# SJTU-ViSYS-team/Avoid-MPC

Hardware: AMD Instinct MI355X
Metric: MPC steps/sec (50k-pt cloud, N=20, 8 obstacle constraints) (higher is better)
Workload: dtype f64; 1 GPU; BASELINE configs[1] batched as configs[2]: 256 scenes/GPU x (50000-pt obstacle cloud + 5000-pt edge cloud, N=20, K=8), fresh frame + zero warm start every step, every in-flight step on its own frames; scenes_per_gpu=256, points=50000, horizon=20, K=8, mpc_max_iter=3, ipm_max_iter=100, streams_in_flight=10, steps_per_launch=4, scenes_per_launch=1024, distinct_frames_bytes=6758400000, hw_queues=4, tie_order=lowest index, parallelism=single GPU, no process group, rccl=no process group (single GPU, plain run): RCCL not used

## Files before the change

avoid_mpc_amd/capi.py:

```python
import ctypes as C
import os

HERE = os.path.dirname(os.path.abspath(__file__))
LIB_PATH = os.path.join(HERE, "libavoid_mpc_amd.so")

AMK_OK, AMK_ERR_INVALID_ARG, AMK_ERR_HIP, AMK_ERR_NO_DEVICE, AMK_ERR_UNSUPPORTED, AMK_ERR_TIMEOUT = 0, 1, 2, 3, 4, 5
AMK_TIES_LOWEST_INDEX, AMK_TIES_NANOFLANN, AMK_TIES_AUTO = 0, 1, 2
AMK_EXACT_OFF, AMK_EXACT_IN_USE, AMK_EXACT_GAVE_UP, AMK_EXACT_TOO_DEEP = -1, 0, 1, 2
AMK_EXACT_NOT_NEEDED = 3
AMK_MAX_K = 64
AMK_MAX_QUERIES = 64
AMK_MAX_HORIZON = 32
AMK_MAX_OUTER_ITER = 8
AMK_MPC_DEFAULT_MAX_ITER = 100

PLUGIN_FUNCTIONS = ["nlp", "nlp_f", "nlp_g", "nlp_grad_f", "nlp_jac_g", "nlp_hess_l", "nlp_grad"]
PLUGIN_HELPERS = ["alloc_mem", "init_mem", "free_mem", "checkout", "release", "incref", "decref", "n_in", "n_out",
                  "default_in", "name_in", "name_out", "sparsity_in", "sparsity_out", "work"]
PLUGIN_SYMBOLS = [f for f in PLUGIN_FUNCTIONS] + [f + "_" + h for f in PLUGIN_FUNCTIONS for h in PLUGIN_HELPERS] + \
                 ["amk_plugin_configure", "amk_plugin_dims"]

SYMBOLS = [
    "amk_version", "amk_status_string", "amk_last_hip_error", "amk_device_count",
    "amk_kd_create", "amk_kd_destroy", "amk_kd_build", "amk_kd_build_pair", "amk_kd_sizes", "amk_kd_search",
    "amk_kd_build_host", "amk_kd_search_host", "amk_kd_tie_flags", "amk_kd_set_tie_order", "amk_kd_exact_status", "amk_kd_exact_status_host", "amk_kd_keyframe_sweep",
    "amk_kd_keyframe_sweep_host", "amk_kd_points_host",
    "amk_mpc_create", "amk_mpc_destroy", "amk_mpc_horizon", "amk_mpc_nx", "amk_mpc_ref_len",
    "amk_mpc_setup_weights", "amk_mpc_setup_tau", "amk_mpc_setup_gains", "amk_mpc_set_drag_coefficient", "amk_mpc_set_drone_radius",
    "amk_kfmap_pool_bytes", "amk_kfmap_create", "amk_kfmap_destroy", "amk_kfmap_reset", "amk_kfmap_scenes", "amk_kfmap_frames", "amk_kfmap_twc", "amk_kfmap_add_vertex",
    "amk_kfmap_update", "amk_kfmap_step", "amk_kfmap_state_host",
    "amk_kfmap_set_tie_order", "amk_kfmap_tie_order_bytes", "amk_kfmap_exact_status_host",
    "amk_kfmap_query_nearest", "amk_kfmap_nearest_distance", "amk_kfmap_query_nearest_host", "amk_kfmap_nearest_distance_host",
    "amk_kfmap_points_host", "amk_kd_query_frames", "amk_kd_nearest_distance_frames", "amk_kd_query_frames_host",
    "amk_mpc_set_drone_accel_limits", "amk_mpc_set_solver_options", "amk_mpc_set_solve_budget", "amk_mpc_set_precision", "amk_mpc_solve",
    "amk_mpc_get_warm_start", "amk_mpc_set_warm_start", "amk_mpc_reset_warm_start",
    "amk_mpc_solve_host", "amk_mpc_ng", "amk_mpc_jac_nnz", "amk_mpc_hess_nnz", "amk_mpc_jac_sparsity",
    "amk_mpc_hess_sparsity", "amk_mpc_eval", "amk_mpc_eval_host", "amk_mpc_np", "amk_mpc_eval_gamma",
    "amk_mpc_eval_gamma_host", "amk_step_batch", "amk_step_batch_frames", "amk_step_batch_host",
    "amk_pipeline_create", "amk_pipeline_destroy", "amk_pipeline_slots", "amk_pipeline_gang", "amk_pipeline_mpc", "amk_pipeline_kd",
    "amk_pipeline_kfmap",
    "amk_pipeline_stream", "amk_pipeline_submit", "amk_pipeline_wait", "amk_pipeline_query", "amk_pipeline_drain",
    "amk_pipeline_outputs", "amk_pipeline_wait_stream",
    "amk_shard_scene_range", "amk_shard_unique_id", "amk_shard_create", "amk_shard_destroy", "amk_shard_rank",
    "amk_shard_world", "amk_shard_last_rccl_error", "amk_shard_gather", "amk_shard_gather_u", "amk_shard_max", "amk_shard_padded_count",
    "amk_shard_rccl_info", "amk_shard_wait",
    "amk_depth_out_size", "amk_depth_to_cloud", "amk_depth_to_cloud_host",
    "amk_depth_to_edge_cloud", "amk_depth_to_edge_cloud_host",
]


class AmkError(RuntimeError):
    pass


class StepParams(C.Structure):
    _fields_ = [("speed", C.c_double), ("safety_distance", C.c_double),
                ("mpc_max_iter", C.c_int), ("reserved", C.c_int)]


class DepthParams(C.Structure):
    _fields_ = [("pixel2meter", C.c_double), ("depth_min", C.c_double), ("depth_max", C.c_double),
                ("resize_scale", C.c_double), ("fx", C.c_double), ("fy", C.c_double), ("cx", C.c_double),
                ("cy", C.c_double), ("Tbc", C.c_double * 16)]


class TaskParams(C.Structure):
    _fields_ = [("decay", C.c_double), ("iter_time", C.c_double), ("farest_point", C.c_double), ("height", C.c_double),
                ("slow_down_kp", C.c_double), ("slow_down_kd", C.c_double), ("a_max_xy", C.c_double), ("a_max_z", C.c_double),
                ("use_odom_est", C.c_int), ("task", C.c_int)]


class KfmapParams(C.Structure):
    _fields_ = [("max_frame_count", C.c_int), ("keyframe_th_count", C.c_int), ("keyframe_th_dist", C.c_double), ("depth_min", C.c_double),
                ("Tbc", C.c_double * 16)]


class PipelineConfig(C.Structure):
    _fields_ = [("n_slots", C.c_int), ("n_scenes", C.c_int), ("max_points", C.c_int), ("max_edge_points", C.c_int),
                ("T", C.c_double), ("dt", C.c_double), ("nearest_point_num", C.c_int), ("queue_depth", C.c_int),
                ("gang", C.c_int), ("step", StepParams), ("task", TaskParams), ("depth", DepthParams), ("keyframes", KfmapParams)]


class PipelineFrame(C.Structure):
    _fields_ = [("d_cloud", C.c_void_p), ("d_cloud_counts", C.c_void_p), ("d_edge", C.c_void_p), ("d_edge_counts", C.c_void_p),
                ("point_stride", C.c_int), ("keep_warm_start", C.c_int), ("d_state_quad", C.c_void_p), ("d_pos_x", C.c_void_p),
                ("d_ref_path_init", C.c_void_p), ("d_u_out", C.c_void_p), ("d_odom", C.c_void_p), ("odom_age", C.c_double),
                ("d_cmd_out", C.c_void_p), ("d_depth", C.c_void_p), ("depth_type", C.c_int), ("depth_rows", C.c_int), ("depth_cols", C.c_int),
                ("reserved", C.c_int), ("d_Twb", C.c_void_p), ("kf_obstacle", C.c_void_p), ("kf_edge", C.c_void_p), ("n_keyframes", C.c_int),
                ("reserved2", C.c_int), ("d_Twc_cur", C.c_void_p), ("camera", C.c_void_p), ("input_ready", C.c_void_p),
                ("d_global_goal", C.c_void_p)]


class FrameCamera(C.Structure):
    _fields_ = [("fx", C.c_double), ("fy", C.c_double), ("cx", C.c_double), ("cy", C.c_double),
                ("depth_max", C.c_double), ("width", C.c_int), ("height", C.c_int)]


AMK_DEPTH_U16, AMK_DEPTH_F32 = 0, 1

_lib = None


def load():
    global _lib
    if _lib is not None:
        return _lib
    if not os.path.exists(LIB_PATH):
        raise AmkError(f"{LIB_PATH} is missing: build it with `python -m avoid_mpc_amd.build` "
                       "(hipcc, gfx950).  There is no CPU fallback.")
    try:
        import torch
    except ImportError:
        pass
    lib = C.CDLL(LIB_PATH)
    vp, i, d, ll = C.c_void_p, C.c_int, C.c_double, C.c_longlong
    sig = {
        "amk_version": (i, []),
        "amk_status_string": (C.c_char_p, [i]),
        "amk_last_hip_error": (i, []),
        "amk_device_count": (i, []),
        "amk_kd_create": (i, [i, i, C.POINTER(vp)]),
        "amk_kd_destroy": (i, [vp]),
        "amk_kd_build": (i, [vp, vp, i, ll, vp, vp]),
        "amk_kd_build_pair": (i, [vp, vp, vp, vp, vp, vp, i, vp]),
        "amk_kd_sizes": (i, [vp, vp, vp]),
        "amk_kd_search": (i, [vp, vp, i, i, vp, vp, vp, vp, vp]),
        "amk_kd_tie_flags": (i, [vp, vp, i, i, i, vp, vp]),
        "amk_kd_set_tie_order": (i, [vp, i]),
        "amk_kd_exact_status": (i, [vp, vp, vp]),
        "amk_kd_exact_status_host": (i, [vp, vp]),
        "amk_kd_keyframe_sweep": (i, [vp, vp, d, i, vp, vp, vp]),
        "amk_kd_keyframe_sweep_host": (i, [vp, vp, d, i, vp, vp]),
        "amk_kd_points_host": (i, [vp, vp, vp]),
        "amk_kd_build_host": (i, [vp, vp, i, ll, vp]),
        "amk_kd_search_host": (i, [vp, vp, i, i, vp, vp, vp, vp]),
        "amk_mpc_create": (i, [d, d, i, i, C.POINTER(vp)]),
        "amk_mpc_destroy": (i, [vp]),
        "amk_mpc_horizon": (i, [vp]),
        "amk_mpc_nx": (i, [vp]),
        "amk_mpc_ref_len": (i, [vp]),
        "amk_mpc_setup_weights": (i, [vp, vp]),
        "amk_mpc_setup_tau": (i, [vp, vp]),
        "amk_mpc_setup_gains": (i, [vp, vp]),
        "amk_mpc_set_drag_coefficient": (i, [vp, d, d, d]),
        "amk_mpc_set_drone_radius": (i, [vp, d]),
        "amk_mpc_set_drone_accel_limits": (i, [vp, d, d, d, d]),
        "amk_mpc_set_solver_options": (i, [vp, d, i]),
        "amk_mpc_set_precision": (i, [vp, i]),
        "amk_mpc_solve": (i, [vp, vp, vp, vp, vp, i, vp]),
        "amk_mpc_get_warm_start": (i, [vp, vp, vp]),
        "amk_mpc_set_warm_start": (i, [vp, vp, vp]),
        "amk_mpc_reset_warm_start": (i, [vp, vp]),
        "amk_mpc_solve_host": (i, [vp, vp, vp, vp, vp, i]),
        "amk_mpc_ng": (i, [vp]),
        "amk_mpc_jac_nnz": (i, [vp]),
        "amk_mpc_hess_nnz": (i, [vp]),
        "amk_mpc_jac_sparsity": (i, [vp, vp, vp]),
        "amk_mpc_hess_sparsity": (i, [vp, vp, vp]),
        "amk_mpc_eval": (i, [vp, vp, vp, vp, vp, vp, vp, vp, vp, vp]),
        "amk_mpc_eval_host": (i, [vp, vp, vp, vp, vp, vp, vp, vp, vp]),
        "amk_mpc_np": (i, [vp]),
        "amk_mpc_eval_gamma": (i, [vp, vp, vp, vp, vp, vp, vp, vp]),
        "amk_mpc_eval_gamma_host": (i, [vp, vp, vp, vp, vp, vp, vp]),
        "amk_step_batch": (i, [vp, vp, vp, C.POINTER(StepParams), vp, vp, vp, vp, vp, vp, vp]),
        "amk_step_batch_host": (i, [vp, vp, vp, C.POINTER(StepParams), vp, vp, vp, vp, vp, vp]),
        "amk_step_batch_frames": (i, [vp, vp, i, vp, C.POINTER(FrameCamera), vp, C.POINTER(StepParams), vp, vp, vp, vp, vp,
                                      vp, vp]),
        "amk_pipeline_create": (i, [C.POINTER(PipelineConfig), C.POINTER(vp)]),
        "amk_pipeline_destroy": (i, [vp]),
        "amk_pipeline_slots": (i, [vp]),
        "amk_mpc_set_solve_budget": (i, [vp, i, i]),
        "amk_pipeline_gang": (i, [vp]),
        "amk_pipeline_mpc": (vp, [vp, i]),
        "amk_pipeline_kd": (vp, [vp, i, i]),
        "amk_pipeline_kfmap": (vp, [vp, i]),
        "amk_pipeline_stream": (vp, [vp, i]),
        "amk_pipeline_submit": (i, [vp, C.POINTER(PipelineFrame), C.POINTER(i)]),
        "amk_pipeline_wait": (i, [vp, i]),
        "amk_pipeline_wait_stream": (i, [vp, i, vp]),
        "amk__pipeline_inject_failure": (i, [vp, i]),
        "amk_pipeline_query": (i, [vp, i]),
        "amk_pipeline_drain": (i, [vp]),
        "amk_pipeline_outputs": (i, [vp, i, C.POINTER(vp), C.POINTER(vp), C.POINTER(vp), C.POINTER(vp)]),
        "amk_kfmap_pool_bytes": (i, [i, i, i, i, C.POINTER(C.c_longlong)]),
        "amk_kfmap_create": (i, [i, i, i, C.POINTER(KfmapParams), C.POINTER(vp)]),
        "amk_kfmap_destroy": (i, [vp]),
        "amk_kfmap_reset": (i, [vp, i, i, vp]),
        "amk_kfmap_scenes": (i, [vp]),
        "amk_kfmap_frames": (i, [vp]),
        "amk_kfmap_twc": (vp, [vp]),
        "amk_kfmap_add_vertex": (i, [vp, i, i, vp, vp, vp, vp, i, vp, vp]),
        "amk_kfmap_update": (i, [vp, vp]),
        "amk_kfmap_step": (i, [vp, vp, vp, C.POINTER(StepParams), vp, vp, vp, vp, vp, vp, vp]),
        "amk_kfmap_state_host": (i, [vp, vp, vp, vp, vp]),
        "amk_kfmap_set_tie_order": (i, [vp, i]),
        "amk_kfmap_tie_order_bytes": (i, [i, i, i, i, C.POINTER(C.c_longlong)]),
        "amk_kfmap_exact_status_host": (i, [vp, vp, vp]),
        "amk_kfmap_query_nearest": (i, [vp, C.POINTER(FrameCamera), vp, i, i, i, i, vp, vp, vp, vp, vp]),
        "amk_kfmap_nearest_distance": (i, [vp, vp, i, i, vp, vp]),
        "amk_kfmap_query_nearest_host": (i, [vp, C.POINTER(FrameCamera), vp, i, i, i, i, vp, vp, vp, vp]),
        "amk_kfmap_nearest_distance_host": (i, [vp, vp, i, i, vp]),
        "amk_kfmap_points_host": (i, [vp, i, vp, ll, vp, C.POINTER(ll)]),
        "amk_kd_query_frames": (i, [vp, i, vp, C.POINTER(FrameCamera), vp, i, i, i, vp, vp, vp, vp, vp]),
        "amk_kd_nearest_distance_frames": (i, [vp, i, vp, i, i, vp, vp]),
        "amk_kd_query_frames_host": (i, [vp, i, vp, C.POINTER(FrameCamera), vp, i, i, i, vp, vp, vp, vp]),
        "amk_shard_scene_range": (i, [i, i, i, C.POINTER(i), C.POINTER(i)]),
        "amk_shard_unique_id": (i, [C.c_char_p]),
        "amk_shard_create": (i, [C.c_char_p, i, i, C.POINTER(vp)]),
        "amk_shard_destroy": (i, [vp]),
        "amk_shard_rank": (i, [vp]),
        "amk_shard_world": (i, [vp]),
        "amk_shard_last_rccl_error": (i, []),
        "amk_shard_gather": (i, [vp, vp, ll, vp, vp]),
        "amk_shard_gather_u": (i, [vp, vp, i, vp, vp]),
        "amk_shard_max": (i, [vp, vp, i, vp]),
        "amk_shard_padded_count": (i, [i, i]),
        "amk_shard_rccl_info": (i, [C.c_char_p, i, C.POINTER(i), C.POINTER(i)]),
        "amk_shard_wait": (i, [vp, vp, d]),
        "amk_depth_out_size": (i, [i, i, d, C.POINTER(i), C.POINTER(i)]),
        "amk_depth_to_cloud": (i, [vp, i, i, i, C.c_longlong, i, C.POINTER(DepthParams), vp, vp, i, C.c_longlong, vp, vp]),
        "amk_depth_to_cloud_host": (i, [vp, i, i, i, C.c_longlong, i, C.POINTER(DepthParams), vp, vp, i, C.c_longlong, vp]),
        "amk_depth_to_edge_cloud": (i, [vp, i, i, i, C.c_longlong, i, C.POINTER(DepthParams), vp, vp, i, C.c_longlong, vp, vp]),
        "amk_depth_to_edge_cloud_host": (i, [vp, i, i, i, C.c_longlong, i, C.POINTER(DepthParams), vp, vp, i, C.c_longlong, vp]),
    }
    sig["amk__kd_set_mode"] = (i, [vp, i])
    sig["amk__sweep_set_target"] = (None, [i])
    sig["amk__sweep_set_order"] = (None, [i])
    sig["amk__frames_force_wide"] = (None, [i])
    sig["amk__mpc_ref_states"] = (i, [vp, vp, ll])
    sig["amk__kfmap_slots_host"] = (i, [vp, vp, vp, vp, vp, vp])
    for name, (res, args) in sig.items():
        fn = getattr(lib, name, None)
        if fn is None:
# ... 60 lines not shown
```

avoid_mpc_amd/csrc/pipeline.hip:

```cpp
#include "mpc_handle.h"

#include <chrono>
#include <cstdlib>
#include <cstring>
#include <vector>

struct amk_pipeline {
    amk_pipeline_config cfg;
    struct Staged {
        amk_pipeline_frame frame;
        std::vector<amk_kd *> kf_obstacle, kf_edge;
        bool has_camera = false;
        amk_frame_camera camera{};
        hipEvent_t input_ready = nullptr;
    };
    struct Slot {
        hipStream_t stream = nullptr;
        std::vector<hipEvent_t> done;
        long long count = 0;
        long long waited = 0;
        amk_kd *obstacle = nullptr, *edge = nullptr;
        amk_mpc *mpc = nullptr;
        amk::DevBuf<double> ref_path, u, x0array, state_quad, pos_x;
        amk::DevBuf<int> flags;
        std::vector<Staged> open;
        int point_stride = 3;
        amk::DevBuf<float> dcloud, dedge;
        amk::DevBuf<int> dcount, decount;
        amk::DevBuf<double> Twc;
        bool ref_inited[AMK_PIPELINE_MAX_GANG] = {};
        amk_kfmap *map = nullptr;
        int fail_status = AMK_OK;
    };
    int depth = 1, gang = 1;
    std::vector<Slot> slots;
    int next = 0;
    long long submitted = 0;
    int inject_failure = 0;
};

namespace {
struct GatherArgs {
    const double *sq[AMK_PIPELINE_MAX_GANG], *px[AMK_PIPELINE_MAX_GANG], *ref[AMK_PIPELINE_MAX_GANG];
    int keep_warm_start[AMK_PIPELINE_MAX_GANG];
    double *sq_dst, *px_dst, *ref_dst, *w0;
    int n_sq, n_px, n_ref, n_w0;
};
__global__ __launch_bounds__(256) void pipeline_gather_kernel(const GatherArgs a) {
    const int g = blockIdx.y;
    const int stride = gridDim.x * 256, t0 = blockIdx.x * 256 + threadIdx.x;
    if (a.sq_dst && a.sq[g]) {
        for (int i = t0; i < a.n_sq; i += stride) a.sq_dst[(size_t)g * a.n_sq + i] = a.sq[g][i];
        for (int i = t0; i < a.n_px; i += stride) a.px_dst[(size_t)g * a.n_px + i] = a.px[g][i];
    }
    if (a.ref[g])
        for (int i = t0; i < a.n_ref; i += stride) a.ref_dst[(size_t)g * a.n_ref + i] = a.ref[g][i];
    if (!a.keep_warm_start[g])
        for (int i = t0; i < a.n_w0; i += stride) a.w0[(size_t)g * a.n_w0 + i] = 0.0;
}
struct ScatterArgs {
    double *dst[AMK_PIPELINE_MAX_GANG];
    double *cmd[AMK_PIPELINE_MAX_GANG];
    const double *odom[AMK_PIPELINE_MAX_GANG];
    const double *u;
    const int *flags;
    int n_u, S;
    double kp, kd, a_max_xy, a_max_z;
};
__global__ __launch_bounds__(256) void pipeline_scatter_kernel(const ScatterArgs a) {
#pragma clang fp contract(off)
    const int g = blockIdx.y;
    if (a.dst[g] && a.dst[g] != a.u + (size_t)g * a.n_u)
        for (int i = blockIdx.x * 256 + threadIdx.x; i < a.n_u; i += gridDim.x * 256) a.dst[g][i] = a.u[(size_t)g * a.n_u + i];
    if (a.cmd[g]) {
        for (int i = blockIdx.x * 256 + threadIdx.x; i < a.S * 3; i += gridDim.x * 256) {
            const int s = i / 3, c = i - 3 * s;
            const size_t gs = (size_t)g * a.S + s;
            double v;
            if (a.flags[gs * 4 + 0]) v = a.u[gs * 4 + c];
            else {
                const double *o = a.odom[g] + (size_t)s * 10;
                v = -o[4 + c] * a.kp - o[7 + c] * a.kd + (c == 2 ? 9.8 : 0.0);
                const double lim = c == 2 ? a.a_max_z : a.a_max_xy;
                v = fmax(-lim, fmin(lim, v));
            }
            a.cmd[g][i] = v;
        }
    }
}

__global__ __launch_bounds__(256) void pipeline_twc_update_kernel(const double *__restrict__ Twb, const int *__restrict__ counts,
                                                                  double *__restrict__ Twc, int S, const amk_depth_params prm) {
// ... 248 lines not shown
            sa.dst[g] = f.d_u_out; sa.cmd[g] = f.d_odom ? f.d_cmd_out : nullptr; sa.odom[g] = f.d_odom;
            any = any || sa.dst[g] || sa.cmd[g];
        }
        sa.u = s.u.p; sa.flags = s.flags.p; sa.n_u = S * 4; sa.S = S;
        sa.kp = c.task.slow_down_kp; sa.kd = c.task.slow_down_kd; sa.a_max_xy = c.task.a_max_xy; sa.a_max_z = c.task.a_max_z;
        if (any) {
            hipLaunchKernelGGL(pipeline_scatter_kernel, dim3((sa.n_u + 255) / 256 > 16 ? 16 : (sa.n_u + 255) / 256, filled), dim3(256), 0, st, sa);
            AMK_HIP(hipGetLastError());
        }
    }
    AMK_HIP(hipEventRecord(s.done[s.count % p->depth], st));
    ++s.count;
    for (int g = 0; g < filled; ++g)
        if (frame(g).d_odom && frame(g).d_ref_path_init) s.ref_inited[g] = true;
    s.open.clear();
    return AMK_OK;
}
int launch_gang(amk_pipeline *p, Slot &s) {
    const int filled = (int)s.open.size();
    if (filled > p->gang || filled > AMK_PIPELINE_MAX_GANG) return AMK_ERR_INVALID_ARG;
    if ((s.map || !s.open[0].kf_obstacle.empty()) && ((s.obstacle && s.obstacle->tie_order == AMK_TIES_AUTO) || (s.edge && s.edge->tie_order == AMK_TIES_AUTO)))
        return AMK_ERR_UNSUPPORTED;
    Launch L{p, p->cfg, s, p->gang, p->cfg.n_scenes, amk_mpc_horizon(s.mpc), p->cfg.step.mpc_max_iter, filled, s.stream};
    int rc;
    if ((rc = L.wait_for_inputs()) != AMK_OK) return rc;
    if ((rc = L.restart_robots()) != AMK_OK) return rc;
    if ((rc = L.gather_inputs()) != AMK_OK) return rc;
    if (p->inject_failure == 1) { p->inject_failure = 0; return AMK_ERR_HIP; }
    if ((rc = L.depth_stage()) != AMK_OK) return rc;
    Stopwatch watch;
    if ((rc = L.build_indices(watch)) != AMK_OK) return rc;
    if (p->inject_failure == 2) { p->inject_failure = 0; return AMK_ERR_HIP; }
    rc = L.control_step();
    if (Stopwatch::on())
        fprintf(stderr, "amk_pipeline launch: add_vertex %.0f us, map update %.0f us, step %.0f us (host enqueue time)\n", watch.us[0],
                watch.us[1], watch.lap(2));
    return rc != AMK_OK ? rc : L.finish();
}
int launch_slot(amk_pipeline *p, Slot &s) {
    if (s.open.empty()) return AMK_OK;
    Stopwatch watch;
    const int st = launch_gang(p, s);
    if (Stopwatch::on()) fprintf(stderr, "amk_pipeline launch_gang total: %.0f us (host)\n", watch.lap());
    if (st != AMK_OK) {
        for (bool &b : s.ref_inited) b = false;
        s.open.clear();
        (void)hipEventRecord(s.done[s.count % p->depth], s.stream);
        ++s.count;
    }
    s.fail_status = st;
    if (&s == &p->slots[p->next]) p->next = (p->next + 1) % (int)p->slots.size();
    return st;
}
int create_slot(const amk_pipeline *p, Slot &s) {
    const amk_pipeline_config &cfg = p->cfg;
    const int GS = p->gang * cfg.n_scenes;
    AMK_HIP(hipStreamCreateWithFlags(&s.stream, hipStreamNonBlocking));
    s.done.assign(p->depth, nullptr);
    for (auto &ev : s.done) AMK_HIP(hipEventCreateWithFlags(&ev, hipEventDisableTiming));
    int st;
    if ((st = amk_kd_create(GS, cfg.max_points, &s.obstacle)) != AMK_OK) return st;
    if ((st = amk_kd_create(GS, cfg.max_edge_points, &s.edge)) != AMK_OK) return st;
    if ((st = amk_mpc_create(cfg.T, cfg.dt, cfg.nearest_point_num, GS, &s.mpc)) != AMK_OK) return st;
    if (cfg.keyframes.max_frame_count > 0) {
        amk_kfmap_params kp = cfg.keyframes;
        auto all_zero = [](const double *T) { bool z = true; for (int e = 0; e < 16; ++e) z = z && T[e] == 0.0; return z; };
        if (all_zero(kp.Tbc)) std::memcpy(kp.Tbc, cfg.depth.Tbc, sizeof kp.Tbc);
        if (all_zero(kp.Tbc)) kp.Tbc[0] = kp.Tbc[5] = kp.Tbc[10] = kp.Tbc[15] = 1.0;
        if ((st = amk_kfmap_create(GS, cfg.max_points, cfg.max_edge_points, &kp, &s.map)) != AMK_OK) return st;
    }
    const size_t S = GS, N = amk_mpc_horizon(s.mpc);
    AMK_HIP(alloc_all(s.ref_path, S * N * 10, s.u, S * 4, s.x0array, S * N * 14, s.flags, S * 4, s.state_quad, S * cfg.step.mpc_max_iter * 10, s.pos_x, S));
    return AMK_OK;
}
int frame_args(const amk_pipeline_config &c, const amk_pipeline_frame *f) {
    if (f->d_depth) {
        if (!f->d_Twb || f->depth_rows <= 0 || f->depth_cols <= 0 || (f->depth_type != AMK_DEPTH_U16 && f->depth_type != AMK_DEPTH_F32))
            return AMK_ERR_INVALID_ARG;
        int w = 0, h = 0;
        if (amk_depth_out_size(f->depth_rows, f->depth_cols, c.depth.resize_scale, &w, &h) != AMK_OK) return AMK_ERR_INVALID_ARG;
        if ((long long)w * h > c.max_points || (long long)w * h > c.max_edge_points) return AMK_ERR_INVALID_ARG;
        if ((long long)w * h > AMK_EDGE_MAX_PIXELS) return AMK_ERR_UNSUPPORTED;
    } else if (!f->d_cloud || !f->d_edge) return AMK_ERR_INVALID_ARG;
    if (!f->d_odom && (!f->d_state_quad || !f->d_pos_x || !f->d_ref_path_init)) return AMK_ERR_INVALID_ARG;
    return (f->n_keyframes < 0 || f->n_keyframes > AMK_MAX_FRAMES - 1) ? AMK_ERR_INVALID_ARG : AMK_OK;
}
amk_pipeline::Staged staged(const amk_pipeline_frame &f) {
    amk_pipeline::Staged o;
    o.frame = f;
    if (f.n_keyframes > 0) {
        o.kf_obstacle.assign(f.kf_obstacle, f.kf_obstacle + f.n_keyframes);
        o.kf_edge.assign(f.kf_edge, f.kf_edge + f.n_keyframes);
    }
    o.has_camera = f.camera != nullptr;
    if (f.camera) o.camera = *f.camera;
    o.input_ready = (hipEvent_t)f.input_ready;
    o.frame.kf_obstacle = o.frame.kf_edge = nullptr; o.frame.camera = nullptr;
    return o;
}
}

extern "C" {
int amk_pipeline_create(const amk_pipeline_config *cfg, amk_pipeline **out) {
    if (!cfg || !out || cfg->n_slots <= 0 || cfg->n_slots > AMK_PIPELINE_MAX_SLOTS || cfg->n_scenes <= 0 ||
        cfg->max_points <= 0 || cfg->max_edge_points <= 0 || cfg->gang < 0 || cfg->gang > AMK_PIPELINE_MAX_GANG ||
        cfg->step.mpc_max_iter < 1 || cfg->step.mpc_max_iter > AMK_MAX_OUTER_ITER || cfg->keyframes.max_frame_count < 0 ||
        (cfg->task.task != AMK_TASK_FORWARD && cfg->task.task != AMK_TASK_GLOBAL_GOAL))
        return AMK_ERR_INVALID_ARG;
    *out = nullptr;
    if (amk_device_count() <= 0) return AMK_ERR_NO_DEVICE;
    amk_pipeline *p = new amk_pipeline();
    p->cfg = *cfg;
    p->depth = cfg->queue_depth > 0 ? cfg->queue_depth : AMK_PIPELINE_DEFAULT_DEPTH;
    if (p->depth > AMK_PIPELINE_MAX_DEPTH) p->depth = AMK_PIPELINE_MAX_DEPTH;
    p->gang = cfg->gang > 0 ? cfg->gang : 1;
    p->slots.resize(cfg->n_slots);
    for (auto &s : p->slots)
        if (const int st = create_slot(p, s); st != AMK_OK) {
            amk_pipeline_destroy(p);
            return st;
        }
    *out = p;
    return AMK_OK;
}

int amk_pipeline_destroy(amk_pipeline *p) {
    if (!p) return AMK_ERR_INVALID_ARG;
    for (auto &s : p->slots) {
        if (s.stream) (void)hipStreamSynchronize(s.stream);
        if (s.obstacle) amk_kd_destroy(s.obstacle);
        if (s.edge) amk_kd_destroy(s.edge);
        if (s.mpc) amk_mpc_destroy(s.mpc);
        if (s.map) amk_kfmap_destroy(s.map);
        for (auto ev : s.done)
            if (ev) (void)hipEventDestroy(ev);
        if (s.stream) (void)hipStreamDestroy(s.stream);
    }
    delete p;
    return AMK_OK;
}

int amk_pipeline_slots(const amk_pipeline *p) { return p ? (int)p->slots.size() : -1; }
int amk_pipeline_gang(const amk_pipeline *p) { return p ? p->gang : -1; }
amk_mpc *amk_pipeline_mpc(amk_pipeline *p, int slot) { const Slot *s = slot_at(p, slot); return s ? s->mpc : nullptr; }
amk_kfmap *amk_pipeline_kfmap(amk_pipeline *p, int slot) { const Slot *s = slot_at(p, slot); return s ? s->map : nullptr; }
void *amk_pipeline_stream(amk_pipeline *p, int slot) { const Slot *s = slot_at(p, slot); return s ? (void *)s->stream : nullptr; }
amk_kd *amk_pipeline_kd(amk_pipeline *p, int slot, int which) {
    const Slot *s = slot_at(p, slot);
    return !s ? nullptr : (which == 0 ? s->obstacle : (which == 1 ? s->edge : nullptr));
}

int amk_pipeline_submit(amk_pipeline *p, const amk_pipeline_frame *f, int *ticket_out) {
    if (!p || !f) return AMK_ERR_INVALID_ARG;
    if (const int st = frame_args(p->cfg, f); st != AMK_OK) return st;
    const int si = p->next, ns = (int)p->slots.size();
    Slot &s = p->slots[si];
    if (s.map && (f->n_keyframes > 0 || (!f->d_depth && (!f->d_Twc_cur || !f->camera)))) return AMK_ERR_INVALID_ARG;
    if (s.map && !s.open.empty()) {
        const amk_pipeline::Staged &o = s.open[0];
        if ((o.frame.d_depth != nullptr) != (f->d_depth != nullptr)) return AMK_ERR_INVALID_ARG;
        if (f->d_depth && (o.frame.depth_rows != f->depth_rows || o.frame.depth_cols != f->depth_cols)) return AMK_ERR_INVALID_ARG;
        if (!f->d_depth && std::memcmp(&o.camera, f->camera, sizeof(amk_frame_camera)) != 0) return AMK_ERR_INVALID_ARG;
    }
    if (f->n_keyframes > 0) {
        if (p->gang != 1) return AMK_ERR_UNSUPPORTED;
        if (!f->kf_obstacle || !f->kf_edge) return AMK_ERR_INVALID_ARG;
        for (int i = 0; i < f->n_keyframes; ++i)
            if (!f->kf_obstacle[i] || !f->kf_edge[i]) return AMK_ERR_INVALID_ARG;
    }
    if (f->d_odom && !f->d_ref_path_init && !s.ref_inited[s.open.size() < AMK_PIPELINE_MAX_GANG ? s.open.size() : 0]) return AMK_ERR_INVALID_ARG;
    const int stride = f->d_depth ? 3 : (f->point_stride ? f->point_stride : 3);
    if (stride != 3 && stride != 4) return AMK_ERR_INVALID_ARG;
    if (!s.open.empty() && stride != s.point_stride) return AMK_ERR_INVALID_ARG;
    if ((int)s.open.size() >= p->gang) return AMK_ERR_INVALID_ARG;
    if (s.open.empty() && s.count - s.waited >= p->depth) {
        Stopwatch watch;
// ... 3 lines not shown
        if (ws != AMK_OK) return ws;
        s.waited = s.count - p->depth + 1;
    }
    const int g = (int)s.open.size();
    s.point_stride = stride;
    s.open.push_back(staged(*f));
    if (ticket_out) *ticket_out = g * ns + si;
    ++p->submitted;
    if ((int)s.open.size() == p->gang) return launch_slot(p, s);
    return AMK_OK;
}

int amk_pipeline_wait(amk_pipeline *p, int ticket) {
    Slot *s = slot_of(p, ticket);
    if (!s) return AMK_ERR_INVALID_ARG;
    if (const int st = launch_slot(p, *s); st != AMK_OK) return st;
    if (s->waited < s->count) {
        if (const int ws = wait_event(s->done[(s->count - 1) % p->depth]); ws != AMK_OK) return ws;
        s->waited = s->count;
    }
    return s->fail_status;
}

int amk_pipeline_wait_stream(amk_pipeline *p, int ticket, void *stream) {
    Slot *s = slot_of(p, ticket);
    if (!s) return AMK_ERR_INVALID_ARG;
    if (const int st = launch_slot(p, *s); st != AMK_OK) return st;
    if (s->count > 0) AMK_HIP(hipStreamWaitEvent((hipStream_t)stream, s->done[(s->count - 1) % p->depth], 0));
    return s->fail_status;
}

int amk_pipeline_query(amk_pipeline *p, int ticket) {
    Slot *s = slot_of(p, ticket);
    if (!s) return -1;
    if (!s->open.empty()) return 0;
    if (s->fail_status != AMK_OK) return -1;
    if (s->waited >= s->count) return 1;
    const hipError_t e = hipEventQuery(s->done[(s->count - 1) % p->depth]);
    if (e == hipSuccess) { s->waited = s->count; return 1; }
    return e == hipErrorNotReady ? 0 : -1;
}

int amk_pipeline_drain(amk_pipeline *p) {
    if (!p) return AMK_ERR_INVALID_ARG;
    int first_error = AMK_OK;
    for (auto &s : p->slots)
        if (const int st = launch_slot(p, s); st != AMK_OK && first_error == AMK_OK) first_error = st;
    for (int i = 0; i < (int)p->slots.size(); ++i)
        if (const int st = amk_pipeline_wait(p, i); st != AMK_OK && first_error == AMK_OK) first_error = st;
    return first_error;
}

int amk__pipeline_inject_failure(amk_pipeline *p, int stage) {
    if (!p || stage < 0 || stage > 2) return AMK_ERR_INVALID_ARG;
    p->inject_failure = stage;
    return AMK_OK;
}

int amk_pipeline_outputs(amk_pipeline *p, int ticket, double **d_u, double **d_x0array, int **d_flags, double **d_ref_path) {
    Slot *s = slot_of(p, ticket);
    if (!s) return AMK_ERR_INVALID_ARG;
    const size_t S = p->cfg.n_scenes, N = amk_mpc_horizon(s->mpc), o = (size_t)(ticket / (int)p->slots.size()) * S;
    if (d_u) *d_u = s->u.p + o * 4;
    if (d_x0array) *d_x0array = s->x0array.p + o * N * 14;
    if (d_flags) *d_flags = s->flags.p + o * 4;
    if (d_ref_path) *d_ref_path = s->ref_path.p + o * N * 10;
    return AMK_OK;
}
}
```

avoid_mpc_amd/csrc/probe.hip:

```cpp
#include "amk_common.h"

namespace {
constexpr int kCopyThreads = 256;
typedef float v4f __attribute__((ext_vector_type(4)));
template <int UNROLL, bool NT>
__global__ __launch_bounds__(kCopyThreads) void hbm_copy_kernel(const v4f *__restrict__ src, v4f *__restrict__ dst, size_t n16) {
    const size_t stride = (size_t)gridDim.x * kCopyThreads;
    size_t i = (size_t)blockIdx.x * kCopyThreads + threadIdx.x;
    for (; i + (UNROLL - 1) * stride < n16; i += UNROLL * stride) {
        v4f v[UNROLL];
#pragma unroll
        for (int u = 0; u < UNROLL; ++u) v[u] = NT ? __builtin_nontemporal_load(src + i + u * stride) : src[i + u * stride];
#pragma unroll
        for (int u = 0; u < UNROLL; ++u) {
            if (NT) __builtin_nontemporal_store(v[u], dst + i + u * stride);
            else dst[i + u * stride] = v[u];
        }
    }
    for (; i < n16; i += stride) dst[i] = src[i];
}

template <bool NT>
__global__ __launch_bounds__(kCopyThreads) void hbm_copy_flat_kernel(const v4f *__restrict__ src, v4f *__restrict__ dst, size_t n16) {
    const size_t i = (size_t)blockIdx.x * kCopyThreads + threadIdx.x;
    if (i >= n16) return;
    const v4f v = src[i];
    if (NT) __builtin_nontemporal_store(v, dst + i);
    else dst[i] = v;
}

template <bool NT>
int time_copy_flat(const void *d_src, void *d_dst, size_t n16, int reps, hipStream_t stream, double *ms_out) {
    const size_t nblk = (n16 + kCopyThreads - 1) / kCopyThreads;
    if (nblk > 0x7fffffffull) return AMK_ERR_UNSUPPORTED;
    hipEvent_t e0, e1;
    AMK_HIP(hipEventCreate(&e0));
    AMK_HIP(hipEventCreate(&e1));
    hipLaunchKernelGGL((hbm_copy_flat_kernel<NT>), dim3((unsigned)nblk), dim3(kCopyThreads), 0, stream, (const v4f *)d_src, (v4f *)d_dst, n16);
    AMK_HIP(hipEventRecord(e0, stream));
    for (int r = 0; r < reps; ++r)
        hipLaunchKernelGGL((hbm_copy_flat_kernel<NT>), dim3((unsigned)nblk), dim3(kCopyThreads), 0, stream, (const v4f *)d_src, (v4f *)d_dst, n16);
    AMK_HIP(hipEventRecord(e1, stream));
    AMK_HIP(hipEventSynchronize(e1));
    float ms = 0.f;
    AMK_HIP(hipEventElapsedTime(&ms, e0, e1));
    (void)hipEventDestroy(e0);
    (void)hipEventDestroy(e1);
    AMK_HIP(hipGetLastError());
    *ms_out = (double)ms / reps;
    return AMK_OK;
}

template <int UNROLL, bool NT>
int time_copy(const void *d_src, void *d_dst, size_t n16, int blocks, int reps, hipStream_t stream, double *ms_out) {
    hipEvent_t e0, e1;
    AMK_HIP(hipEventCreate(&e0));
    AMK_HIP(hipEventCreate(&e1));
    hipLaunchKernelGGL((hbm_copy_kernel<UNROLL, NT>), dim3(blocks), dim3(kCopyThreads), 0, stream, (const v4f *)d_src, (v4f *)d_dst, n16);
    AMK_HIP(hipEventRecord(e0, stream));
    for (int r = 0; r < reps; ++r)
        hipLaunchKernelGGL((hbm_copy_kernel<UNROLL, NT>), dim3(blocks), dim3(kCopyThreads), 0, stream, (const v4f *)d_src, (v4f *)d_dst, n16);
    AMK_HIP(hipEventRecord(e1, stream));
    AMK_HIP(hipEventSynchronize(e1));
    float ms = 0.f;
    AMK_HIP(hipEventElapsedTime(&ms, e0, e1));
    (void)hipEventDestroy(e0);
    (void)hipEventDestroy(e1);
    AMK_HIP(hipGetLastError());
    *ms_out = (double)ms / reps;
    return AMK_OK;
}
}

extern "C" int amk__hbm_copy_probe(const void *d_src, void *d_dst, size_t n_bytes, int reps, void *stream_, double *ms_out, int *variant_out) {
    if (!d_src || !d_dst || n_bytes < 16 || (n_bytes & 15) || reps < 1 || !ms_out) return AMK_ERR_INVALID_ARG;
    hipStream_t stream = (hipStream_t)stream_;
    int dev = 0, cus = 256;
    AMK_HIP(hipGetDevice(&dev));
    AMK_HIP(hipDeviceGetAttribute(&cus, hipDeviceAttributeMultiprocessorCount, dev));
    const size_t n16 = n_bytes / 16;
    double best = 1e30;
    int best_v = 0;
    for (int bpc : {8, 16, 32}) {
        const int blocks = cus * bpc;
        double ms = 0.0;
        int st;
#define AMK_TRY(U, NT)                                                                   \
        st = time_copy<U, NT>(d_src, d_dst, n16, blocks, reps, stream, &ms);           \
        if (st != AMK_OK) return st;                                                     \
        if (ms < best) { best = ms; best_v = U * 1000 + (NT ? 100 : 0) + bpc; }
        AMK_TRY(2, false) AMK_TRY(4, false) AMK_TRY(8, false) AMK_TRY(2, true) AMK_TRY(4, true) AMK_TRY(8, true)
#undef AMK_TRY
    }
    for (int nt = 0; nt < 2; ++nt) {
        double ms = 0.0;
        const int st = nt ? time_copy_flat<true>(d_src, d_dst, n16, reps, stream, &ms) : time_copy_flat<false>(d_src, d_dst, n16, reps, stream, &ms);
        if (st != AMK_OK) return st;
        if (ms < best) { best = ms; best_v = 1 + 100 * nt; }
    }
    *ms_out = best;
    if (variant_out) *variant_out = best_v;
    return AMK_OK;
}
```

avoid_mpc_amd/host.py:

```python
import ctypes as C

import numpy as np
import torch

from . import capi


def _dev():
    if not torch.cuda.is_available():
        raise capi.AmkError("no GPU visible: the hot path has no CPU fallback")
    return torch.device("cuda", torch.cuda.current_device())


class KdBatch:
    def __init__(self, n_scenes, max_points, handle=None):
        self.lib = capi.load()
        self.S, self.max_points = int(n_scenes), int(max_points)
        self.owned = handle is None
        if handle is None:
            handle = C.c_void_p()
            capi.check(self.lib.amk_kd_create(self.S, self.max_points, C.byref(handle)), "amk_kd_create")
        self.h = handle if isinstance(handle, C.c_void_p) else C.c_void_p(handle)

    def close(self):
# ... 363 lines not shown
        self._events = []
        self._max_points = (int(max_points), int(max_edge_points))
        hs = n_scenes * self.gang
        self._mpc = [MpcBatch(prm.T, prm.dt, prm.K, hs, handle=self.lib.amk_pipeline_mpc(h, i)) for i in range(n_slots)]
        self._kd = [(KdBatch(hs, max_points, handle=self.lib.amk_pipeline_kd(h, i, 0)),
                     KdBatch(hs, max_edge_points, handle=self.lib.amk_pipeline_kd(h, i, 1))) for i in range(n_slots)]
        for m in self._mpc:
            m.configure(prm)

    @staticmethod
    def _kfmap_params(keyframes):
        if not keyframes:
            return capi.KfmapParams()
        kp = capi.KfmapParams(int(keyframes["max_frame_count"]), int(keyframes["th_count"]), float(keyframes["th_dist"]),
                              float(keyframes["depth_min"]))
        if keyframes.get("Tbc") is not None:
            T = np.asarray(keyframes["Tbc"], np.float64).reshape(16)
            for i in range(16):
                kp.Tbc[i] = float(T[i])
        return kp

    def kfmap_state(self, slot):
        h = self.lib.amk_pipeline_kfmap(self.h, int(slot))
        assert h, "the pipeline was created without keyframes"
        S = self.S * self.gang
        F = self.lib.amk_kfmap_frames(h)
        nk = np.zeros(S, np.int32); nq = np.zeros(S, np.int32); out = np.zeros(S, np.int32); sz = np.zeros((S, F), np.int32)
        capi.check(self.lib.amk_kfmap_state_host(h, nk.ctypes.data_as(C.c_void_p), nq.ctypes.data_as(C.c_void_p),
                                                 out.ctypes.data_as(C.c_void_p), sz.ctypes.data_as(C.c_void_p)), "amk_kfmap_state_host")
        return dict(n_keyframes=nk, n_query_frames=nq, last_outliers=out, frame_sizes=sz)

    def kfmap(self, slot):
        h = self.lib.amk_pipeline_kfmap(self.h, int(slot))
        assert h, "the pipeline was created without keyframes"
        return KfMap(0, self._max_points[0], self._max_points[1], 0, 0, 0, 0, None, handle=h)

    def kfmap_query(self, slot, queries, k=None, cam=None, edge=False, after_wait=False):
        m = self.kfmap(slot)
        Q = int(queries.shape[1])
        out = torch.empty((m.S, Q), dtype=torch.float64, device=queries.device) if k is None else _query_out(m.S, Q, int(k), queries.device)
        run = (lambda st: m.nearest_distance(queries, stream=st, out=out)) if k is None else \
              (lambda st: m.query_nearest(queries, k, cam=cam, edge=edge, stream=st, out=out))
        if after_wait:
            return run(None)
        raw = self.lib.amk_pipeline_stream(self.h, int(slot))
        ext = torch.cuda.ExternalStream(int(raw))
        ext.wait_stream(torch.cuda.current_stream())
        run(int(raw))
        torch.cuda.current_stream().wait_stream(ext)
        return out

    def kfmap_points(self, slot, scene):
        return self.kfmap(slot).points(scene)

    def mpc(self, slot):
        return self._mpc[slot]

    def kd(self, slot, which):
        return self._kd[slot][which]

    def close(self):
        if getattr(self, "h", None):
            self.lib.amk_pipeline_destroy(self.h)
            self.h = None

    __del__ = close

    def submit(self, clouds, edges, state_quad=None, pos_x=None, ref_path_init=None, cloud_counts=None, edge_counts=None, u_out=None,
               keep_warm_start=False, order_after_current_stream=True, odom=None, odom_age=0.0, cmd_out=None, depth=None, Twb=None,
               keyframes=None, Twc_cur=None, cam=None, global_goal=None):
        opt = lambda t: t.data_ptr() if t is not None else None
        dinfo = (None, 0, 0, 0, 0, None)
        if depth is not None:
            assert depth.dim() == 3 and depth.is_contiguous() and Twb.dtype == torch.float64 and Twb.is_contiguous()
            kind = capi.AMK_DEPTH_F32 if depth.dtype == torch.float32 else capi.AMK_DEPTH_U16
            dinfo = (depth.data_ptr(), kind, int(depth.shape[1]), int(depth.shape[2]), 0, Twb.data_ptr())
        else:
            assert clouds.dtype == torch.float32 and edges.dtype == torch.float32 and clouds.shape[2] == edges.shape[2]
        self._kf_keep = (None, None, cam)
        kinfo = (None, None, 0, 0, opt(Twc_cur), C.cast(C.pointer(cam), C.c_void_p) if cam is not None else None)
        if keyframes:
            ko = (C.c_void_p * len(keyframes))(*[k[0].h for k in keyframes]); ke = (C.c_void_p * len(keyframes))(*[k[1].h for k in keyframes])
            self._kf_keep = (ko, ke, cam)
            kinfo = (C.cast(ko, C.c_void_p), C.cast(ke, C.c_void_p), len(keyframes), 0) + kinfo[4:]
        ev_ptr = None
        if order_after_current_stream:
            ev = torch.cuda.Event()
            ev.record(torch.cuda.current_stream())
            ev_ptr = ev.cuda_event
            self._events.append(ev)
            if len(self._events) > 4 * self.n_slots * self.gang + 8:
                del self._events[:len(self._events) // 2]
        fr = capi.PipelineFrame(opt(clouds), opt(cloud_counts), opt(edges), opt(edge_counts),
                                int(clouds.shape[2]) if clouds is not None else 3, int(bool(keep_warm_start)), opt(state_quad), opt(pos_x),
                                opt(ref_path_init), opt(u_out), opt(odom), float(odom_age), opt(cmd_out), *dinfo, *kinfo, ev_ptr,
                                opt(global_goal))
        slot = C.c_int(-1)
        capi.check(self.lib.amk_pipeline_submit(self.h, C.byref(fr), C.byref(slot)), "amk_pipeline_submit")
        return slot.value

    def wait_stream(self, ticket, stream=None):
        capi.check(self.lib.amk_pipeline_wait_stream(self.h, int(ticket), capi.stream_ptr(stream)), "amk_pipeline_wait_stream")

    def output_tensors(self, ticket):
        ptr = [C.c_void_p() for _ in range(4)]
        capi.check(self.lib.amk_pipeline_outputs(self.h, int(ticket), *[C.byref(p) for p in ptr]), "amk_pipeline_outputs")
# ... 129 lines not shown
```

include/avoid_mpc_amd.h:

```cpp
#ifndef AVOID_MPC_AMD_H
#define AVOID_MPC_AMD_H

#ifdef __cplusplus
extern "C" {
#endif

typedef enum amk_status {
    AMK_OK = 0,
    AMK_ERR_INVALID_ARG = 1,
    AMK_ERR_HIP = 2,
    AMK_ERR_NO_DEVICE = 3,
    AMK_ERR_UNSUPPORTED = 4,
    AMK_ERR_TIMEOUT = 5
} amk_status;

#define AMK_MAX_K 64
#define AMK_MAX_QUERIES 64
#define AMK_MAX_HORIZON 32
#define AMK_S_DIM 10
#define AMK_U_DIM 4
#define AMK_MPC_DEFAULT_MAX_ITER 100
#define AMK_MAX_BUDGET_ROUNDS 16

int amk_version(void);
// ... 95 lines not shown
    double speed;
    double safety_distance;
    int mpc_max_iter;
    int reserved;
} amk_step_params;

#define AMK_MAX_OUTER_ITER 8

int amk_step_batch(amk_kd *obstacle, amk_kd *edge, amk_mpc *mpc, const amk_step_params *params,
                   const double *d_state_quad, const double *d_pos_x, double *d_ref_path,
                   double *d_u, double *d_x0array, int *d_flags, void *stream);

#define AMK_MAX_FRAMES 16
#define AMK_MAX_MAP_FRAMES 101
typedef struct amk_frame_camera {
    double fx, fy, cx, cy;
    double depth_max;
    int width, height;
} amk_frame_camera;
int amk_step_batch_frames(amk_kd *const *obstacle, amk_kd *const *edge, int n_frames, const double *d_Twc,
                          const amk_frame_camera *cam, amk_mpc *mpc, const amk_step_params *params,
                          const double *d_state_quad, const double *d_pos_x, double *d_ref_path, double *d_u,
                          double *d_x0array, int *d_flags, void *stream);

int amk_step_batch_host(amk_kd *obstacle, amk_kd *edge, amk_mpc *mpc, const amk_step_params *params,
                        const double *h_state_quad, const double *h_pos_x, double *h_ref_path,
                        double *h_u, double *h_x0array, int *h_flags);

typedef struct amk_pipeline amk_pipeline;
typedef struct amk_depth_params {
    double pixel2meter;
    double depth_min;
    double depth_max;
    double resize_scale;
    double fx, fy, cx, cy;
    double Tbc[16];
} amk_depth_params;
typedef struct amk_task_params {
    double decay;
    double iter_time;
    double farest_point;
    double height;
    double slow_down_kp, slow_down_kd;
    double a_max_xy, a_max_z;
    int use_odom_est;
    int task;
} amk_task_params;
#define AMK_TASK_FORWARD 0
#define AMK_TASK_GLOBAL_GOAL 1
#define AMK_PIPELINE_MAX_SLOTS 64
#define AMK_PIPELINE_DEFAULT_DEPTH 3
#define AMK_PIPELINE_MAX_DEPTH 64
#define AMK_PIPELINE_MAX_GANG 8
typedef struct amk_kfmap amk_kfmap;
typedef struct amk_kfmap_params {
    int max_frame_count;
    int keyframe_th_count;
    double keyframe_th_dist;
    double depth_min;
    double Tbc[16];
} amk_kfmap_params;
typedef struct amk_pipeline_config {
    int n_slots;
    int n_scenes;
    int max_points;
    int max_edge_points;
    double T, dt;
    int nearest_point_num;
    int queue_depth;
    int gang;
    amk_step_params step;
    amk_task_params task;
    amk_depth_params depth;
    amk_kfmap_params keyframes;
} amk_pipeline_config;
typedef struct amk_pipeline_frame {
    const float *d_cloud;
    const int *d_cloud_counts;
    const float *d_edge;
    const int *d_edge_counts;
    int point_stride;
    int keep_warm_start;
    const double *d_state_quad;
    const double *d_pos_x;
    const double *d_ref_path_init;
    double *d_u_out;
    const double *d_odom;
    double odom_age;
    double *d_cmd_out;
    const void *d_depth;
    int depth_type, depth_rows, depth_cols, reserved;
    const double *d_Twb;
    amk_kd *const *kf_obstacle;
    amk_kd *const *kf_edge;
    int n_keyframes, reserved2;
    const double *d_Twc_cur;
    const struct amk_frame_camera *camera;
    void *input_ready;
    const double *d_global_goal;
} amk_pipeline_frame;
int amk_pipeline_create(const amk_pipeline_config *cfg, amk_pipeline **out);
int amk_pipeline_destroy(amk_pipeline *p);
int amk_pipeline_slots(const amk_pipeline *p);
int amk_pipeline_gang(const amk_pipeline *p);
amk_mpc *amk_pipeline_mpc(amk_pipeline *p, int slot);
amk_kd *amk_pipeline_kd(amk_pipeline *p, int slot, int which );
amk_kfmap *amk_pipeline_kfmap(amk_pipeline *p, int slot);
void *amk_pipeline_stream(amk_pipeline *p, int slot);
int amk_pipeline_submit(amk_pipeline *p, const amk_pipeline_frame *frame, int *ticket_out);
int amk_pipeline_wait(amk_pipeline *p, int ticket);
int amk_pipeline_wait_stream(amk_pipeline *p, int ticket, void *stream);
int amk_pipeline_query(amk_pipeline *p, int ticket);
int amk_pipeline_drain(amk_pipeline *p);
int amk_pipeline_outputs(amk_pipeline *p, int ticket, double **d_u, double **d_x0array, int **d_flags, double **d_ref_path);

int amk_kfmap_pool_bytes(int n_scenes, int max_points, int max_edge_points, int max_frame_count, long long *bytes_out);
int amk_kfmap_create(int n_scenes, int max_points, int max_edge_points, const amk_kfmap_params *prm, amk_kfmap **out);
int amk_kfmap_destroy(amk_kfmap *map);
int amk_kfmap_reset(amk_kfmap *map, int first_scene, int n_scenes, void *stream);
int amk_kfmap_scenes(const amk_kfmap *map);
int amk_kfmap_frames(const amk_kfmap *map);
const double *amk_kfmap_twc(const amk_kfmap *map);
int amk_kfmap_add_vertex(amk_kfmap *map, int first_scene, int n_scenes, const float *d_xyz, const int *d_counts,
                         const float *d_edge_xyz, const int *d_edge_counts, int point_stride, const double *d_Twc, void *stream);
int amk_kfmap_update(amk_kfmap *map, void *stream);
int amk_kfmap_step(amk_kfmap *map, const struct amk_frame_camera *cam, amk_mpc *mpc, const amk_step_params *prm,
                   const double *d_state_quad, const double *d_pos_x, double *d_ref_path, double *d_u, double *d_x0array,
                   int *d_flags, void *stream);
int amk_kfmap_state_host(amk_kfmap *map, int *h_n_keyframes, int *h_n_query_frames, int *h_last_outliers, int *h_frame_sizes);
int amk_kfmap_set_tie_order(amk_kfmap *map, int mode);
int amk_kfmap_tie_order_bytes(int n_scenes, int max_points, int max_edge_points, int max_frame_count, long long *bytes_out);
int amk_kfmap_exact_status_host(amk_kfmap *map, int *h_obs, int *h_edge);

int amk_kfmap_query_nearest(amk_kfmap *map, const struct amk_frame_camera *cam, const double *d_queries, int query_stride,
                            int n_queries, int k, int query_edge, float *d_pts, double *d_sqdist, int *d_frame,
                            int *d_counts, void *stream);
int amk_kfmap_nearest_distance(amk_kfmap *map, const double *d_queries, int query_stride, int n_queries,
                               double *d_dist, void *stream);
int amk_kfmap_query_nearest_host(amk_kfmap *map, const struct amk_frame_camera *cam, const double *h_queries, int query_stride,
                                 int n_queries, int k, int query_edge, float *h_pts, double *h_sqdist, int *h_frame,
                                 int *h_counts);
int amk_kfmap_nearest_distance_host(amk_kfmap *map, const double *h_queries, int query_stride, int n_queries, double *h_dist);
int amk_kfmap_points_host(amk_kfmap *map, int scene, float *h_xyz, long long capacity_points, int *h_frame_sizes,
                          long long *n_points_out);
int amk_kd_query_frames(amk_kd *const *frames, int n_frames, const double *d_Twc, const struct amk_frame_camera *cam,
                        const double *d_queries, int query_stride, int n_queries, int k, float *d_pts, double *d_sqdist,
                        int *d_frame, int *d_counts, void *stream);
int amk_kd_nearest_distance_frames(amk_kd *const *frames, int n_frames, const double *d_queries, int query_stride,
                                   int n_queries, double *d_dist, void *stream);
int amk_kd_query_frames_host(amk_kd *const *frames, int n_frames, const double *h_Twc, const struct amk_frame_camera *cam,
                             const double *h_queries, int query_stride, int n_queries, int k, float *h_pts, double *h_sqdist,
                             int *h_frame, int *h_counts);

typedef struct amk_shard amk_shard;
#define AMK_SHARD_ID_BYTES 128
int amk_shard_scene_range(int rank, int world, int total, int *first, int *count);
int amk_shard_unique_id(char *id_out );
// ... 38 lines not shown
```

Baseline: 429,500 MPC steps/s.

## Create pipeline streams with distinct priorities when HW queues are scarce

When the HIP hardware queue pool (GPU_MAX_HW_QUEUES, default 4) is smaller than the number of pipeline slots, each slot's stream is created with hipStreamCreateWithPriority, spread across the available priority classes. The aim is to give more in-flight slots their own hardware queues so they stop serialising on a few pooled queues. It adds an env override, a fallback to plain streams, a queue-mode query and an overlap probe kernel for testing. Priority queues may change scheduling fairness, and the runtime might still map them onto shared queues.

```diff
diff --git a/avoid_mpc_amd/capi.py b/avoid_mpc_amd/capi.py
--- a/avoid_mpc_amd/capi.py
+++ b/avoid_mpc_amd/capi.py
@@ -38,7 +38,7 @@
     "amk_mpc_hess_sparsity", "amk_mpc_eval", "amk_mpc_eval_host", "amk_mpc_np", "amk_mpc_eval_gamma",
     "amk_mpc_eval_gamma_host", "amk_step_batch", "amk_step_batch_frames", "amk_step_batch_host",
     "amk_pipeline_create", "amk_pipeline_destroy", "amk_pipeline_slots", "amk_pipeline_gang", "amk_pipeline_mpc", "amk_pipeline_kd",
-    "amk_pipeline_kfmap",
+    "amk_pipeline_kfmap", "amk_pipeline_queue_mode",
     "amk_pipeline_stream", "amk_pipeline_submit", "amk_pipeline_wait", "amk_pipeline_query", "amk_pipeline_drain",
     "amk_pipeline_outputs", "amk_pipeline_wait_stream",
     "amk_shard_scene_range", "amk_shard_unique_id", "amk_shard_create", "amk_shard_destroy", "amk_shard_rank",
@@ -97,6 +97,8 @@
 
 
 AMK_DEPTH_U16, AMK_DEPTH_F32 = 0, 1
+AMK_QUEUES_POOLED, AMK_QUEUES_PRIORITY = 0, 1
+AMK_PIPELINE_MAX_OWN_QUEUES = 24
 
 _lib = None
 
@@ -178,7 +180,10 @@
         "amk_pipeline_submit": (i, [vp, C.POINTER(PipelineFrame), C.POINTER(i)]),
         "amk_pipeline_wait": (i, [vp, i]),
         "amk_pipeline_wait_stream": (i, [vp, i, vp]),
+        "amk_pipeline_queue_mode": (i, [vp, i]),
         "amk__pipeline_inject_failure": (i, [vp, i]),
+        "amk__pipeline_queue_policy": (i, [i, i, i, i, vp, vp]),
+        "amk__pipeline_overlap_probe": (i, [vp, i, vp]),
         "amk_pipeline_query": (i, [vp, i]),
         "amk_pipeline_drain": (i, [vp]),
         "amk_pipeline_outputs": (i, [vp, i, C.POINTER(vp), C.POINTER(vp), C.POINTER(vp), C.POINTER(vp)]),
diff --git a/avoid_mpc_amd/csrc/pipeline.hip b/avoid_mpc_amd/csrc/pipeline.hip
--- a/avoid_mpc_amd/csrc/pipeline.hip
+++ b/avoid_mpc_amd/csrc/pipeline.hip
@@ -16,6 +16,7 @@
     };
     struct Slot {
         hipStream_t stream = nullptr;
+        int queue_mode = AMK_QUEUES_POOLED;
         std::vector<hipEvent_t> done;
         long long count = 0;
         long long waited = 0;
@@ -38,6 +39,7 @@
     long long submitted = 0;
     int inject_failure = 0;
 };
+extern "C" int amk__pipeline_queue_policy(int pool, int n_slots, int n_classes, int forced, int *mode_out, int *class_out);
 
 namespace {
 struct GatherArgs {
@@ -392,10 +394,35 @@
     if (&s == &p->slots[p->next]) p->next = (p->next + 1) % (int)p->slots.size();
     return st;
 }
-int create_slot(const amk_pipeline *p, Slot &s) {
+int env_int(const char *name, int absent) {
+    const char *e = std::getenv(name);
+    const int v = e ? std::atoi(e) : 0;
+    return v > 0 ? v : absent;
+}
+int forced_queue_mode() {
+    const char *e = std::getenv("AMK_PIPELINE_QUEUES");
+    if (!e) return -1;
+    return !std::strcmp(e, "pooled") ? AMK_QUEUES_POOLED : !std::strcmp(e, "priority") ? AMK_QUEUES_PRIORITY : -1;
+}
+int g_fail_queue_creation = 0;
+int create_stream(Slot &s, int mode, int priority, bool fail) {
+    s.stream = nullptr;
+    s.queue_mode = AMK_QUEUES_POOLED;
+    if (mode == AMK_QUEUES_PRIORITY) {
+        if (!fail && hipStreamCreateWithPriority(&s.stream, hipStreamNonBlocking, priority) == hipSuccess) {
+            s.queue_mode = AMK_QUEUES_PRIORITY;
+            return AMK_OK;
+        }
+        (void)hipGetLastError();
+        s.stream = nullptr;
+    }
+    AMK_HIP(hipStreamCreateWithFlags(&s.stream, hipStreamNonBlocking));
+    return AMK_OK;
+}
+int create_slot(const amk_pipeline *p, Slot &s, int queue_mode, int priority, bool fail_queue) {
     const amk_pipeline_config &cfg = p->cfg;
     const int GS = p->gang * cfg.n_scenes;
-    AMK_HIP(hipStreamCreateWithFlags(&s.stream, hipStreamNonBlocking));
+    if (const int st = create_stream(s, queue_mode, priority, fail_queue); st != AMK_OK) return st;
     s.done.assign(p->depth, nullptr);
     for (auto &ev : s.done) AMK_HIP(hipEventCreateWithFlags(&ev, hipEventDisableTiming));
     int st;
@@ -455,13 +482,40 @@
     if (p->depth > AMK_PIPELINE_MAX_DEPTH) p->depth = AMK_PIPELINE_MAX_DEPTH;
     p->gang = cfg->gang > 0 ? cfg->gang : 1;
     p->slots.resize(cfg->n_slots);
-    for (auto &s : p->slots)
-        if (const int st = create_slot(p, s); st != AMK_OK) {
+    int least = 0, greatest = 0;
+    if (hipDeviceGetStreamPriorityRange(&least, &greatest) != hipSuccess || least < greatest) least = greatest = 0;
+    int mode[AMK_PIPELINE_MAX_SLOTS], cls[AMK_PIPELINE_MAX_SLOTS];
+    amk__pipeline_queue_policy(env_int("GPU_MAX_HW_QUEUES", 4), cfg->n_slots, least - greatest + 1, forced_queue_mode(), mode, cls);
+    const bool fail_queue = g_fail_queue_creation != 0;
+    g_fail_queue_creation = 0;
+    for (int i = 0; i < cfg->n_slots; ++i)
+        if (const int st = create_slot(p, p->slots[i], mode[i], greatest + cls[i], fail_queue); st != AMK_OK) {
             amk_pipeline_destroy(p);
             return st;
         }
     *out = p;
     return AMK_OK;
+}
+
+int amk__pipeline_queue_policy(int pool, int n_slots, int n_classes, int forced, int *mode_out, int *class_out) {
+    if (pool < 1 || n_slots < 1 || !mode_out || !class_out) return -1;
+    if (n_classes < 1) n_classes = 1;
+    int mode = forced;
+    if (mode != AMK_QUEUES_POOLED && mode != AMK_QUEUES_PRIORITY)
+        mode = (pool >= n_slots + 1 || pool >= AMK_PIPELINE_MAX_OWN_QUEUES) ? AMK_QUEUES_POOLED : AMK_QUEUES_PRIORITY;
+    int own = 0;
+    if (mode == AMK_QUEUES_PRIORITY) own = (int)std::min<long long>(std::min(n_slots, AMK_PIPELINE_MAX_OWN_QUEUES), (long long)n_classes * pool);
+    const int normal = (n_classes - 1) / 2;
+    for (int i = 0; i < n_slots; ++i) {
+        mode_out[i] = i < own ? AMK_QUEUES_PRIORITY : AMK_QUEUES_POOLED;
+        const int k = i % n_classes;
+        class_out[i] = i < own ? (k < n_classes - normal ? normal + k : n_classes - 1 - k) : normal;
+    }
+    return own;
+}
+
+int amk_pipeline_queue_mode(const amk_pipeline *p, int slot) {
+    return (p && slot >= 0 && slot < (int)p->slots.size()) ? p->slots[slot].queue_mode : -1;
 }
 
 int amk_pipeline_destroy(amk_pipeline *p) {
@@ -571,6 +625,7 @@
 }
 
 int amk__pipeline_inject_failure(amk_pipeline *p, int stage) {
+    if (!p && stage == 3) { g_fail_queue_creation = 1; return AMK_OK; }
     if (!p || stage < 0 || stage > 2) return AMK_ERR_INVALID_ARG;
     p->inject_failure = stage;
     return AMK_OK;
diff --git a/avoid_mpc_amd/csrc/probe.hip b/avoid_mpc_amd/csrc/probe.hip
--- a/avoid_mpc_amd/csrc/probe.hip
+++ b/avoid_mpc_amd/csrc/probe.hip
@@ -70,6 +70,39 @@
     *ms_out = (double)ms / reps;
     return AMK_OK;
 }
+
+__global__ __launch_bounds__(64) void overlap_probe_kernel(unsigned long long *__restrict__ start_end, unsigned *__restrict__ sink, int iters, unsigned seed) {
+    const unsigned long long t0 = wall_clock64();
+    unsigned x = seed + threadIdx.x;
+    for (int i = 0; i < iters; ++i) {
+        x ^= x >> 7;
+        x = x * 1664525u + 1013904223u;
+    }
+    const unsigned long long t1 = wall_clock64();
+    if (threadIdx.x == 0) {
+        start_end[0] = t0;
+        start_end[1] = t1;
+    }
+    sink[threadIdx.x] = x;
+}
+}
+
+extern "C" int amk__pipeline_overlap_probe(amk_pipeline *p, int iters, unsigned long long *h_start_end) {
+    const int n = amk_pipeline_slots(p);
+    if (n <= 0 || iters < 1 || iters > 50000000 || !h_start_end) return AMK_ERR_INVALID_ARG;
+    amk::DevBuf<unsigned long long> d_t;
+    amk::DevBuf<unsigned> d_sink;
+    AMK_HIP(d_t.alloc((size_t)n * 2));
+    AMK_HIP(d_sink.alloc((size_t)n * 64));
+    for (int pass = 0; pass < 2; ++pass) {
+        for (int i = 0; i < n; ++i)
+            hipLaunchKernelGGL(overlap_probe_kernel, dim3(1), dim3(64), 0, (hipStream_t)amk_pipeline_stream(p, i), d_t.p + 2 * i, d_sink.p + 64 * i,
+                               pass ? iters : 16, 12345u + i);
+        AMK_HIP(hipGetLastError());
+        AMK_HIP(hipDeviceSynchronize());
+    }
+    AMK_HIP(hipMemcpy(h_start_end, d_t.p, (size_t)n * 2 * sizeof(unsigned long long), hipMemcpyDeviceToHost));
+    return AMK_OK;
 }
 
 extern "C" int amk__hbm_copy_probe(const void *d_src, void *d_dst, size_t n_bytes, int reps, void *stream_, double *ms_out, int *variant_out) {
diff --git a/avoid_mpc_amd/host.py b/avoid_mpc_amd/host.py
--- a/avoid_mpc_amd/host.py
+++ b/avoid_mpc_amd/host.py
@@ -439,6 +439,9 @@
 
     def kfmap_points(self, slot, scene):
         return self.kfmap(slot).points(scene)
+
+    def queue_mode(self, slot):
+        return self.lib.amk_pipeline_queue_mode(self.h, int(slot))
 
     def mpc(self, slot):
         return self._mpc[slot]
diff --git a/include/avoid_mpc_amd.h b/include/avoid_mpc_amd.h
--- a/include/avoid_mpc_amd.h
+++ b/include/avoid_mpc_amd.h
@@ -171,6 +171,9 @@
 #define AMK_PIPELINE_DEFAULT_DEPTH 3
 #define AMK_PIPELINE_MAX_DEPTH 64
 #define AMK_PIPELINE_MAX_GANG 8
+#define AMK_PIPELINE_MAX_OWN_QUEUES 24
+#define AMK_QUEUES_POOLED 0
+#define AMK_QUEUES_PRIORITY 1
 typedef struct amk_kfmap amk_kfmap;
 typedef struct amk_kfmap_params {
     int max_frame_count;
@@ -222,6 +225,7 @@
 int amk_pipeline_destroy(amk_pipeline *p);
 int amk_pipeline_slots(const amk_pipeline *p);
 int amk_pipeline_gang(const amk_pipeline *p);
+int amk_pipeline_queue_mode(const amk_pipeline *p, int slot);
 amk_mpc *amk_pipeline_mpc(amk_pipeline *p, int slot);
 amk_kd *amk_pipeline_kd(amk_pipeline *p, int slot, int which );
 amk_kfmap *amk_pipeline_kfmap(amk_pipeline *p, int slot);
```

Measured after the change: 509,400 MPC steps/s, median of 6. +18.6%, better.
